# NSLab-CUK/LiteralKG

Measured on AMD Instinct MI355X. Metric: kg_edges_aggregated_per_sec, higher is better.
Workload: dtype f32

## Files before the change

include/literalkg_hip.h:

```cpp
#ifndef LITERALKG_HIP_H
#define LITERALKG_HIP_H

#include <stdint.h>

#ifdef __cplusplus
extern "C" {
#endif

typedef enum {
    LKG_OK = 0,
    LKG_ERR_INVALID_ARG = -1,
    LKG_ERR_HIP = -2,
    LKG_ERR_UNSUPPORTED = -3,
    LKG_ERR_NOMEM = -4
} lkg_status;

int lkg_version(void);
const char *lkg_last_error(void);
int lkg_preload(void);

int lkg_csr_build(int64_t n_entities, int64_t n_edges, const int64_t *h, const int64_t *t,
                  const int64_t *r, int32_t *rowptr, int32_t *col, int32_t *eptr, int32_t *rel,
                  int64_t *order, int64_t *nnz_out);

// ... 148 lines not shown

int lkg_gate_blend_fwd_f32(int64_t n, int32_t d, const float *x, int64_t ldx, const float *gpre,
                           int64_t ldg, const float *zpre, int64_t ldz, float *out, int64_t ldo,
                           void *stream);
int lkg_gate_blend_bwd_f32(int64_t n, int32_t d, const float *x, int64_t ldx, const float *gpre,
                           int64_t ldg, const float *zpre, int64_t ldz, const float *g_out,
                           int64_t ldgo, float *g_x, int64_t ldgx, float *g_gpre, int64_t ldgg,
                           float *g_zpre, int64_t ldgz, int32_t activated, float *g_pre_rowmax, void *stream);

int lkg_gate_blend_bwd_stats_f32(int64_t n, int32_t d, const float *x, int64_t ldx, const float *gpre, int64_t ldg,
                                 const float *zpre, int64_t ldz, const float *g_out, int64_t ldgo, float *g_x,
                                 int64_t ldgx, float *g_gpre, int64_t ldgg, float *g_zpre, int64_t ldgz,
                                 int32_t activated, float *g_pre_rowmax, const float *w, int64_t ldw, int32_t n_w,
                                 float *workspace, int64_t workspace_floats, float *stats, void *stream);

int lkg_gemm_wgrad_f32(int64_t m, int64_t n, int64_t k, const float *a, int64_t lda, const float *a_colmax,
                       const float *b, int64_t ldb, const float *b_colmax, float *c, int64_t ldc, void *stream);
int lkg_gemm_longk_ok(int64_t m, int64_t n, int64_t k, const float *a, int64_t lda, const float *b, int64_t ldb);
int lkg_gemm_longk_f32(int64_t m, int64_t n, int64_t k, const float *a, int64_t lda, const float *b, int64_t ldb,
                       float *c, int64_t ldc, void *stream);
int lkg_gemm_smallm_ok(int64_t m, int64_t n, int64_t k, const float *a, int64_t lda, const float *b, int64_t ldb);
int lkg_gemm_smallm_f32(int64_t m, int64_t n, int64_t k, const float *a, int64_t lda, const float *b, int64_t ldb,
                        float *c, int64_t ldc, void *stream);

int64_t lkg_narrow_layer_bwd_workspace(int64_t n);
int lkg_narrow_layer_bwd_ok(int64_t n, int32_t d_in, int32_t d_out, const float *x, int64_t ldx, const float *z, int64_t ldz,
                            const float *y, int64_t ldy, const float *g_y, int64_t ldgy, const float *g_yn, int64_t ldgyn);
int lkg_narrow_layer_bwd_f32(int64_t n, int32_t d_in, int32_t d_out, const float *x, int64_t ldx, const float *w, int64_t ldw,
                             const float *z, int64_t ldz, float slope, const float *gamma, const float *y, int64_t ldy,
                             const float *save_mean, const float *save_rstd, const float *g_y, int64_t ldgy,
                             const float *g_yn, int64_t ldgyn, float norm_eps, float drop_p, uint64_t seed,
                             const uint8_t *g_yn_rows, float *g_x, int64_t ldgx, float *g_w, float *g_bias,
                             float *g_gamma, float *g_beta, float *workspace, int64_t workspace_floats, void *stream);
int lkg_gemm_skinny_ok(int64_t m, int64_t n, int64_t k, const float *a, int64_t lda, const float *c, int64_t ldc);
int lkg_gemm_skinny_f32(int64_t m, int64_t n, int64_t k, const float *a, int64_t lda, const float *b, int64_t ldb,
                        int32_t trans_b, float beta, float *c, int64_t ldc, const float *bias, void *stream);
int lkg_col_absmax_f32(int64_t n, int32_t d, const float *x, int64_t ldx, float *out, void *stream);

int lkg_colsum_f32(int64_t n, int32_t d, const float *x, int64_t ldx, float *out, void *stream);
int lkg_colsum_weighted_f32(int64_t n, int32_t d, const float *x, int64_t ldx, const float *w, int64_t ldw,
                            int32_t n_w, float *out_sum, float *out_w, int64_t ld_out_w, void *stream);

int lkg_bi_mix_fwd_f32(int64_t n, int32_t d, const float *ego, int64_t lde, const float *side, int64_t lds,
                       const float *h0p, int64_t ldh, float alpha, float *out_sum, int64_t ldos, float *out_prod,
                       int64_t ldop, void *stream);
int lkg_bi_mix_bwd_f32(int64_t n, int32_t d, const float *ego, int64_t lde, const float *side, int64_t lds,
                       const float *g_sum, int64_t ldgs, const float *g_prod, int64_t ldgp, int32_t has_h0, float alpha,
                       float *g_ego, float *g_side, float *g_h0p, void *stream);

int lkg_eltwise_f32(int32_t op, int64_t n, int32_t d, const float *a, int64_t lda, const float *b,
                    int64_t ldb, float alpha, float beta, float *out, int64_t ldo, void *stream);

int lkg_adam_step_f32(int64_t n, float *param, const float *grad, float *exp_avg, float *exp_avg_sq,
                      float lr, float beta1, float beta2, float eps, float weight_decay, int64_t step,
                      void *stream);

int64_t lkg_gemm_workspace(int32_t trans_a, int64_t m, int64_t n, int64_t k);
int lkg_gemm_f32_engine(int32_t trans_a, int32_t trans_b, int64_t m, int64_t n, int64_t k, int64_t workspace_bytes);

int lkg_gemm_f64acc_f32(int32_t trans_a, int32_t trans_b, int64_t m, int64_t n, int64_t k, const float *a, int64_t lda,
                        const float *b, int64_t ldb, float *c, int64_t ldc, void *stream);
int lkg_gemm_f32(int32_t trans_a, int32_t trans_b, int64_t m, int64_t n, int64_t k, float alpha,
                 const float *a, int64_t lda, const float *b, int64_t ldb, float beta, float *c,
                 int64_t ldc, const float *bias, void *workspace, int64_t workspace_bytes, void *stream);

int lkg_row_absmax_f32(int64_t n, int32_t d, const float *x, int64_t ldx, float *out, int32_t accumulate,
// ... 78 lines not shown
```

literalkg_amd/_native.py:

```python
import ctypes as C
import os

_LIB_PATH = os.path.join(os.path.dirname(os.path.abspath(__file__)), "lib", "liblkg_hip.so")
_lib = None

i64, i32, f32, vp, u64 = C.c_int64, C.c_int32, C.c_float, C.c_void_p, C.c_uint64

PROTOTYPES = {
    "lkg_version": [],
    "lkg_last_error": [],
    "lkg_preload": [],
    "lkg_csr_build": [i64, i64, vp, vp, vp, vp, vp, vp, vp, vp, vp],
    "lkg_csr_transpose": [i64, i64, i64, vp, vp, vp, vp, vp],
    "lkg_row_partition": [i64, vp, i32, vp],
    "lkg_csr_coo_indices_i64": [i64, i64, vp, vp, vp, vp],
    "lkg_csr_build_device_workspace": [i64, i64],
    "lkg_csr_build_device": [i64, i64, vp, vp, vp, vp, vp, vp, vp, vp, vp, vp, i64, vp],
    "lkg_csr_transpose_device_workspace": [i64, i64],
    "lkg_csr_transpose_device": [i64, i64, i64, vp, vp, vp, vp, vp, vp, i64, vp],
    "lkg_triples_count": [C.c_char_p, vp],
    "lkg_triples_read": [C.c_char_p, i64, vp, vp, vp, vp],
    "lkg_triples_dedup": [i64, vp, vp, vp, vp, vp],
    "lkg_laplacian_f32": [i64, i64, i64, vp, vp, vp, vp, i32, vp],
    "lkg_laplacian_device_f32": [i64, i64, i32, vp, vp, vp, vp, i32, vp, vp, vp],
# ... 30 lines not shown
                                  vp, f32, u64, vp, vp, i32, vp, i64, vp],
    "lkg_dot_score_fwd_f32": [i64, i32, vp, i64, vp, vp, vp, vp, vp, vp, vp, vp],
    "lkg_dot_score_bwd_f32": [i64, i32, vp, i64, vp, vp, vp, vp, vp, f32, vp, vp, i64, vp],
    "lkg_relu_batchnorm_fwd_f32": [i64, i32, vp, i64, vp, vp, f32, i32, f32, vp, vp, vp, i64, vp, vp, vp],
    "lkg_relu_batchnorm_bwd_f32": [i64, i32, vp, i64, vp, vp, vp, i32, vp, i64, vp, i64, vp, vp, vp],
    "lkg_gate_blend_fwd_f32": [i64, i32, vp, i64, vp, i64, vp, i64, vp, i64, vp],
    "lkg_gate_blend_bwd_f32": [i64, i32, vp, i64, vp, i64, vp, i64, vp, i64, vp, i64, vp, i64, vp, i64, i32, vp, vp],
    "lkg_gate_blend_bwd_stats_f32": [i64, i32, vp, i64, vp, i64, vp, i64, vp, i64, vp, i64, vp, i64, vp, i64, i32, vp, vp,
                                     i64, i32, vp, i64, vp, vp],
    "lkg_row_absmax_f32": [i64, i32, vp, i64, vp, i32, vp],
    "lkg_gemm_tall_workspace": [i32, i32, vp, i32],
    "lkg_gemm_tall_f32": [i64, i32, i32, vp, vp, vp, vp, i32, vp, vp, i32, f32, f32, vp, i64, vp, i32, vp, i64, vp, i64,
                          vp, i64, vp, i64, vp],
    "lkg_linear_act_layernorm_workspace": [i32, i32, vp],
    "lkg_linear_act_layernorm_fwd_f32": [i64, i32, i32, vp, vp, vp, vp, vp, vp, vp, f32, vp, vp, f32, vp, i64, vp, i64, f32,
                                         vp, vp, f32, u64, vp, i64, vp],
    "lkg_gemm_workspace": [i32, i64, i64, i64],
    "lkg_gemm_f32_engine": [i32, i32, i64, i64, i64, i64],
    "lkg_gemm_f32": [i32, i32, i64, i64, i64, f32, vp, i64, vp, i64, f32, vp, i64, vp, vp, i64, vp],
    "lkg_gemm_f64acc_f32": [i32, i32, i64, i64, i64, vp, i64, vp, i64, vp, i64, vp],
    "lkg_colsum_f32": [i64, i32, vp, i64, vp, vp],
    "lkg_col_absmax_f32": [i64, i32, vp, i64, vp, vp],
    "lkg_gemm_longk_ok": [i64, i64, i64, vp, i64, vp, i64],
    "lkg_gemm_longk_f32": [i64, i64, i64, vp, i64, vp, i64, vp, i64, vp],
    "lkg_gemm_smallm_ok": [i64, i64, i64, vp, i64, vp, i64],
    "lkg_gemm_skinny_ok": [i64, i64, i64, vp, i64, vp, i64],
    "lkg_gemm_skinny_f32": [i64, i64, i64, vp, i64, vp, i64, i32, f32, vp, i64, vp, vp],
    "lkg_gemm_smallm_f32": [i64, i64, i64, vp, i64, vp, i64, vp, i64, vp],
    "lkg_gemm_wgrad_f32": [i64, i64, i64, vp, i64, vp, vp, i64, vp, vp, i64, vp],
    "lkg_narrow_layer_bwd_ok": [i64, i32, i32, vp, i64, vp, i64, vp, i64, vp, i64, vp, i64],
    "lkg_narrow_layer_bwd_workspace": [i64],
    "lkg_narrow_layer_bwd_f32": [i64, i32, i32, vp, i64, vp, i64, vp, i64, f32, vp, vp, i64, vp, vp, vp, i64, vp, i64, f32, f32,
                                 u64, vp, vp, i64, vp, vp, vp, vp, vp, i64, vp],
    "lkg_colsum_weighted_f32": [i64, i32, vp, i64, vp, i64, i32, vp, vp, i64, vp],
    "lkg_eltwise_f32": [i32, i64, i32, vp, i64, vp, i64, f32, f32, vp, i64, vp],
    "lkg_bi_mix_fwd_f32": [i64, i32, vp, i64, vp, i64, vp, i64, f32, vp, i64, vp, i64, vp],
    "lkg_bi_mix_bwd_f32": [i64, i32, vp, i64, vp, i64, vp, i64, vp, i64, i32, f32, vp, vp, vp, vp],
    "lkg_adam_step_f32": [i64, vp, vp, vp, vp, f32, f32, f32, f32, f32, i64, vp],
    "lkg_rank_sqnorm_f32": [i64, i32, vp, i64, vp, vp],
    "lkg_rank_queries_f32": [i64, i32, vp, i64, vp, vp, i64, vp, f32, vp, i64, vp],
    "lkg_rank_prepare_f32": [i64, i64, i32, vp, i64, vp, i64, vp, vp, vp, vp, vp, vp, vp, vp, vp, vp, vp, vp],
    "lkg_rank_count_f32": [i64, i64, i32, vp, i64, vp, i64, vp, vp, vp, vp, vp, vp],
    "lkg_topk_splits": [i64, i64, i32],
    "lkg_topk_select_f32": [i64, i64, i32, vp, i64, vp, i64, vp, vp, vp, vp, vp, vp, vp, vp, i32, i32, vp, vp, vp],
    "lkg_topk_merge_f32": [i64, i32, i32, vp, vp, vp, vp, vp, vp, vp],
    "lkg_pair_mlp_scores_f32": [i64, i64, vp, i64, vp, i64, vp, vp, vp, vp, vp, i64, vp],
    "lkg_pair_mlp_splits": [i64, i64, i32],
    "lkg_pair_mlp_select_f32": [i64, i64, vp, i64, vp, i64, vp, vp, vp, vp, vp, vp, vp, vp, vp, vp, vp, i32, i32, vp, vp,
                                vp],
    "lkg_pair_mlp_prepare_f32": [i64, i64, vp, i64, vp, i64, vp, vp, vp, vp, vp, i64, vp, vp, vp, vp, vp, vp, vp, vp, vp,
                                 vp, vp],
    "lkg_pair_mlp_count_f32": [i64, i64, vp, i64, vp, i64, vp, vp, vp, vp, vp, vp, vp, vp, vp],
    "lkg_pair_mlp_pairs_f32": [i64, vp, i64, vp, i64, vp, vp, vp, vp, vp, vp, vp, f32, vp, vp, vp],
    "lkg_binary_curve_workspace": [i64],
    "lkg_binary_curve_f32": [i64, vp, vp, vp, vp, vp, i64, vp],
    "lkg_triple_scores_f32": [i64, i32, vp, i64, vp, vp, vp, vp, i64, vp, f32, i32, vp, f32, vp, vp, vp],
    "lkg_threshold_fit_workspace": [i64, i64],
    "lkg_threshold_fit_f32": [i64, i64, vp, vp, vp, i32, vp, vp, vp, i64, vp],
}
_RESTYPE = {"lkg_last_error": C.c_char_p, "lkg_csr_build_device_workspace": C.c_int64,
            "lkg_gemm_tall_workspace": C.c_int64, "lkg_gemm_workspace": C.c_int64,
            "lkg_linear_act_layernorm_workspace": C.c_int64, "lkg_narrow_layer_bwd_workspace": C.c_int64,
            "lkg_csr_transpose_device_workspace": C.c_int64, "lkg_binary_curve_workspace": C.c_int64,
            "lkg_threshold_fit_workspace": C.c_int64}


# ... 70 lines not shown
```

literalkg_amd/csrc/lkg_spmm.hip:

```cpp
#include <stdlib.h>

#include <algorithm>
#include <type_traits>

#include "lkg_common.h"

namespace {

template <typename V>
struct vec_ops;
template <>
struct vec_ops<float4> {
    static constexpr int W = 4;
    static __device__ __forceinline__ float4 zero() { return f4_zero(); }
    static __device__ __forceinline__ void fma(float4 &a, float s, const float4 &x) { f4_fma(a, s, x); }
    static __device__ __forceinline__ float absmax(const float4 &a) {
        return fmaxf(fmaxf(fabsf(a.x), fabsf(a.y)), fmaxf(fabsf(a.z), fabsf(a.w)));
    }
    template <int M>
    static __device__ __forceinline__ void xor_add(float4 &a) {
        a.x = lane_xor_add<M>(a.x);
        a.y = lane_xor_add<M>(a.y);
        a.z = lane_xor_add<M>(a.z);
        a.w = lane_xor_add<M>(a.w);
// ... 229 lines not shown
            }
        }
        const V *csrc = ex.copy_dst ? reinterpret_cast<const V *>(ex.copy_src + (long)row * ex.ld_copy_src) : nullptr;
        V *cdst = ex.copy_dst ? reinterpret_cast<V *>(ex.copy_dst + (long)row * ex.ld_copy_dst) : nullptr;
#pragma unroll
        for (int i = 0; i < CPL; ++i) {
            const int chunk = lane + i * LPE;
            if (FULL || chunk < nchunk) {
                if (own) ops::fma(acc[i], 1.f, own[chunk]);
                if (own2) ops::fma(acc[i], 1.f, own2[chunk]);
#ifndef LKG_SPMM_PLAIN
                if constexpr (std::is_same<V, float4>::value) {
                    typedef float nt4 __attribute__((ext_vector_type(4)));
                    const nt4 nv = {acc[i].x, acc[i].y, acc[i].z, acc[i].w};
                    __builtin_nontemporal_store(nv, reinterpret_cast<nt4 *>(dst + chunk));
                } else {
                    __builtin_nontemporal_store(acc[i], dst + chunk);
                }
#else
                dst[chunk] = acc[i];
#endif
                if (cdst) cdst[chunk] = csrc[chunk];
                rmax = fmaxf(rmax, ops::absmax(acc[i]));
            }
        }
    }
    if (ex.rowmax) {
        rmax = wave_max(rmax);
        if (lane == 0) atomicMax(ex.rowmax + row, __float_as_int(rmax));
    }
}

template <typename V, int LPE, int U, bool FULL>
__global__ __launch_bounds__(256) void spmm_csr_grouped_kernel(int n_rows, int nchunk,
                                                                const int *__restrict__ rowptr,
                                                                const int *__restrict__ col,
                                                                const float *__restrict__ val,
                                                                const float *__restrict__ x, long ldx,
                                                                float *__restrict__ out, long ldo,
                                                                const float *__restrict__ self, long ld_self,
                                                                const int *__restrict__ long_rows, int n_long,
                                                                int long_thresh, SpmmExtra ex) {
    using ops = vec_ops<V>;
    static_assert(LPE <= 32 && LPE % U == 0, "grouped SpMM: 2+ rows per wave, whole U-groups per chunk");
    __shared__ V part[4][LPE];
    const int lane = threadIdx.x & 63, w = threadIdx.x >> 6;
    if ((int)blockIdx.x < n_long) {
        const int row = long_rows[blockIdx.x];
        const int start = __builtin_amdgcn_readfirstlane(rowptr[row]);
        const int end = __builtin_amdgcn_readfirstlane(rowptr[row + 1]);
        V acc[1] = {ops::zero()};
        accumulate_entries<V, LPE, 1, U, FULL>(acc, start, end, w, 4, lane, nchunk, col, val, x, ldx);
        reduce_subgroups<V, LPE>(acc[0]);
        if (lane < LPE) part[w][lane] = acc[0];
        __syncthreads();
        if (w != 0 || lane >= LPE || !(FULL || lane < nchunk)) return;
        V a = part[0][lane];
#pragma unroll
        for (int k = 1; k < 4; ++k) ops::fma(a, 1.f, part[k][lane]);
        if (self) ops::fma(a, 1.f, reinterpret_cast<const V *>(self + (long)row * ld_self)[lane]);
        if (const float *a2 = ex.add2_row(row)) ops::fma(a, 1.f, reinterpret_cast<const V *>(a2)[lane]);
        reinterpret_cast<V *>(out + (long)row * ldo)[lane] = a;
        if (ex.rowmax) atomicMax(ex.rowmax + row, __float_as_int(ops::absmax(a)));
        if (ex.copy_dst)
            reinterpret_cast<V *>(ex.copy_dst + (long)row * ex.ld_copy_dst)[lane] =
                reinterpret_cast<const V *>(ex.copy_src + (long)row * ex.ld_copy_src)[lane];
        return;
    }
    constexpr int RPW = 64 / LPE;
    const int sub = lane / LPE, sl = lane % LPE;
    const int slot = (((int)blockIdx.x - n_long) * 4 + w) * RPW + sub;
    const bool valid = slot < n_rows;
    const int row = valid ? slot : 0;
    int start = 0, len = 0;
    if (valid) {
        start = rowptr[row];
        len = rowptr[row + 1] - start;
    }
    const bool mine = valid && !(n_long > 0 && len > long_thresh);
    if (!mine) len = 0;
    int maxlen = len;
    int spare = len > 0 ? start : -1;
#pragma unroll
    for (int m = LPE; m < 64; m <<= 1) {
        maxlen = max(maxlen, __shfl_xor(maxlen, m, 64));
        spare = max(spare, __shfl_xor(spare, m, 64));
    }
    V acc = ops::zero();
    for (int k = 0; k < maxlen; k += LPE) {
        const int j = k + sl;
        const int jc = len > 0 ? start + min(j, len - 1) : spare;
        const int c = col[jc];
        const float v = j < len ? val[jc] : 0.f;
        const int mcnt = min(LPE, maxlen - k);
        for (int q = 0; q < mcnt; q += U) {
            int cc[U];
            float vv[U];
            V xv[U];
#pragma unroll
            for (int u = 0; u < U; ++u) {
                cc[u] = __shfl(c, sub * LPE + q + u, 64);
                vv[u] = __shfl(v, sub * LPE + q + u, 64);
            }
#pragma unroll
            for (int u = 0; u < U; ++u) {
                const V *src = reinterpret_cast<const V *>(x + (long)cc[u] * ldx);
                xv[u] = FULL ? src[sl] : src[min(sl, nchunk - 1)];
            }
#pragma unroll
            for (int u = 0; u < U; ++u) ops::fma(acc, vv[u], xv[u]);
        }
    }
    const bool writes = mine && (FULL || sl < nchunk);
    if (writes) {
        if (len == 0) acc = ops::zero();
        if (self) ops::fma(acc, 1.f, reinterpret_cast<const V *>(self + (long)row * ld_self)[sl]);
        if (const float *a2 = ex.add2_row(row)) ops::fma(acc, 1.f, reinterpret_cast<const V *>(a2)[sl]);
        reinterpret_cast<V *>(out + (long)row * ldo)[sl] = acc;
        if (ex.copy_dst)
            reinterpret_cast<V *>(ex.copy_dst + (long)row * ex.ld_copy_dst)[sl] =
                reinterpret_cast<const V *>(ex.copy_src + (long)row * ex.ld_copy_src)[sl];
    }
    if (ex.rowmax) {
        const float rm = group_max<LPE>(writes ? ops::absmax(acc) : 0.f);
        if (mine && sl == 0) atomicMax(ex.rowmax + row, __float_as_int(rm));
    }
}

template <int CPL, bool FULL>
__global__ __launch_bounds__(256) void spmm_flagged4_kernel(int n_rows, int nchunk, const int *__restrict__ rowptr,
                                                             const int *__restrict__ col, const float *__restrict__ val,
                                                             const float *__restrict__ x, long ldx,
                                                             float *__restrict__ out, long ldo,
                                                             const float *__restrict__ self, long ld_self, int n_long,
                                                             int long_thresh, SpmmExtra ex) {
    const int lane = threadIdx.x & 63, q = lane >> 4, ql = lane & 15;
    const int task = (int)blockIdx.x * 4 + (threadIdx.x >> 6);
    const int row_q = task * 4 + q;
    int start = 0, len = 0;
    if (row_q < n_rows) {
        start = rowptr[row_q];
        len = rowptr[row_q + 1] - start;
        if (n_long > 0 && len > long_thresh) len = 0;
    }
    int maxlen = len;
    maxlen = max(maxlen, __shfl_xor(maxlen, 16, 64));
    maxlen = max(maxlen, __shfl_xor(maxlen, 32, 64));
    float4 acc[4][CPL];
#pragma unroll
    for (int r = 0; r < 4; ++r)
#pragma unroll
        for (int i = 0; i < CPL; ++i) acc[r][i] = f4_zero();
    unsigned any = 0;
    for (int p = 0; p < maxlen; p += 16) {
        const int j = p + ql;
        const bool in = j < len;
        const int jj = start + (in ? j : 0);
        const int c = len > 0 ? col[jj] : 0;
        unsigned long long m = __ballot(in && ex.x_rows[c] != 0);
// ... 258 lines not shown
        return LKG_OK;
    }
    const int block_cols = (vec && !x_rows) ? 128 : 256;
    const bool grouped_slabs = vec && !x_rows && block_cols / 4 <= LKG_SPMM_GROUPED_CHUNKS;
    if (d > block_cols && d % block_cols == 0 && !grouped_slabs)
        return vec ? dispatch<float4>(n_rows, block_cols / 4, rowptr, col, val, x, ldx, out, ldo, self, ld_self,
                                      long_rows, n_long, long_thresh, d / block_cols, block_cols, ex, s)
                   : dispatch<float>(n_rows, block_cols, rowptr, col, val, x, ldx, out, ldo, self, ld_self, long_rows,
                                     n_long, long_thresh, d / block_cols, block_cols, ex, s);
    for (int c0 = 0; c0 < d; c0 += block_cols) {
        const int dc = min(block_cols, d - c0);
        const SpmmExtra exc{add2 ? add2 + c0 : nullptr, (long)ld_add2, add2 ? add2_rows : nullptr,
                            copy_dst ? copy_src + c0 : nullptr,
                            (long)ld_copy_src, copy_dst ? copy_dst + c0 : nullptr, (long)ld_copy_dst,
                            reinterpret_cast<int *>(rowmax_out), x_rows, self ? self_rows : nullptr, out_rows, ex.row_list, ex.n_list};
        int rc = vec ? dispatch<float4>(n_rows, dc / 4, rowptr, col, val, x + c0, ldx, out + c0, ldo,
                                        self ? self + c0 : nullptr, ld_self, long_rows, n_long, long_thresh, 1, 0, exc, s)
                     : dispatch<float>(n_rows, dc, rowptr, col, val, x + c0, ldx, out + c0, ldo,
                                       self ? self + c0 : nullptr, ld_self, long_rows, n_long, long_thresh, 1, 0, exc, s);
        if (rc != LKG_OK) return rc;
    }
    return LKG_OK;
}

extern "C" int lkg_spmm_csr_f32(int64_t n_rows, int32_t d, const int32_t *rowptr, const int32_t *col,
                                const float *val, const float *x, int64_t ldx, float *out, int64_t ldo,
                                const float *self, int64_t ld_self, const int32_t *long_rows, int32_t n_long,
                                int32_t long_thresh, void *stream) {
    return lkg_spmm_csr_fused_f32(n_rows, d, rowptr, col, val, x, ldx, out, ldo, self, ld_self, nullptr, 0, nullptr,
                                  nullptr, 0, nullptr, 0, nullptr, nullptr, nullptr, nullptr, long_rows, n_long, long_thresh,
                                  nullptr, 0, nullptr, 0, stream);
}

__global__ void permute_kernel(long n, long n_src, const int *__restrict__ perm, const float *__restrict__ src,
                               float *__restrict__ dst) {
    long i = (long)blockIdx.x * blockDim.x + threadIdx.x;
    const long stride = (long)gridDim.x * blockDim.x;
    for (; i < n; i += stride) {
        const long p = perm[i];
        dst[i] = (p >= 0 && p < n_src) ? src[p] : __builtin_nanf("");
    }
}

extern "C" int lkg_permute_f32(int64_t n, const int32_t *perm, int64_t n_src, const float *src, float *dst, void *stream) {
    LKG_REQUIRE(n >= 0 && n_src >= 0, "lkg_permute_f32: negative extent");
    if (n == 0) return LKG_OK;
    LKG_REQUIRE(perm && src && dst, "lkg_permute_f32: null pointer");
    const int64_t blocks = std::min<int64_t>((n + 255) / 256, 256 * 8);
    hipLaunchKernelGGL(permute_kernel, dim3((unsigned)blocks), dim3(256), 0, (hipStream_t)stream, (long)n, (long)n_src, perm,
                       src, dst);
    LKG_CHECK_LAUNCH("lkg_permute_f32");
    return LKG_OK;
}

__global__ __launch_bounds__(256) void csr_check_kernel(long n_rows, const int *__restrict__ rowptr, long nnz,
                                                        const int *__restrict__ col, long col_offset, long n_cols,
                                                        int *__restrict__ bad) {
    const long stride = (long)gridDim.x * blockDim.x;
    const long t0 = (long)blockIdx.x * blockDim.x + threadIdx.x;
    int mine = 0;
    for (long i = t0; i < n_rows; i += stride) {
        const long a = rowptr[i], b = rowptr[i + 1];
        mine += (a < 0 || a > b || b > nnz) ? 1 : 0;
    }
    long lo = rowptr[0], hi = rowptr[n_rows];
    lo = lo < 0 ? 0 : (lo > nnz ? nnz : lo);
// ... 89 lines not shown
```

literalkg_amd/model.py:

```python
from __future__ import annotations

import math
import os
from typing import Optional

import torch
import torch.nn as nn

from . import ops, pruned
from .gate import Gate, GateMul
from .graph import KGStructure


class AttentionCSR:

    def __init__(self, graph: KGStructure, val: torch.Tensor, val_t: Optional[torch.Tensor] = None):
        self.graph = graph
        self.val = val
        self.val_t = val_t if val_t is not None else (
            ops.permute_values(val, graph.t_perm) if graph.t_perm is not None and val.is_cuda else None)

    def aggregate(self, ego: torch.Tensor, plus_self: bool = False, bias: Optional[torch.Tensor] = None) -> torch.Tensor:
        return ops.aggregate(ego, self.graph, self.val, self.val_t, plus_self, bias)

# ... 103 lines not shown
                                  want_y=self.want_output)
        self.last_normalized = yn
        return y

    def _linear_finish(self, xs, ws, bias):
        ln = self.layer_normalize
        if len(xs) == 1 and ops.narrow_layer_ok(xs[0], ws[0]):
            p = float(self.dropout) if self.training else 0.0
            y, yn = ops.narrow_layer(xs[0], ws[0], bias, ln.weight, ln.bias, want_norm=True, drop_p=p, yn_out=self.norm_out,
                                     want_y=self.want_output)
            self.last_normalized = yn
            return y
        if ops.fused_layer_wanted(xs, ws, (bias, ln.weight, ln.bias)):
            p = float(self.dropout) if self.training else 0.0
            y, yn = ops.linear_act_layernorm(xs, ws, bias, ln.weight, ln.bias, want_norm=True, drop_p=p, yn_out=self.norm_out,
                                             want_y=self.want_output)
            self.last_normalized = yn
            return y
        return self._finish(ops.multi_linear(xs, ws, bias))

    def narrows(self) -> bool:
        return self.aggregator_type == "gcn" and not self.use_residual and 2 * self.out_dim <= self.in_dim

    def forward(self, ego_embeddings, A_in: AttentionCSR, all_layers, lamda, alpha, l):
        ego = ego_embeddings
        h0 = all_layers[0]
        kind = self.aggregator_type
        if kind == "gcn":
            att = getattr(A_in, "att", A_in)
            if self.narrows() and isinstance(att, AttentionCSR):
                p = ops.linear(ego, self.linear.weight, None)
                return self._finish(att.aggregate(p, True, bias=self.linear.bias))
            if not self.use_residual:
                return self._linear_finish((A_in.aggregate(ego, True),), (self.linear.weight,), self.linear.bias)
            z = self._res_lin(self.linear, A_in.aggregate(ego, True), h0, lamda, alpha, l)
            return self._finish(z)
        if kind == "gin":
            return self._gin(ego, A_in.aggregate(ego, True), h0, all_layers, lamda, alpha, l)
        side = A_in.aggregate(ego)
        if kind == "graphsage":
            if self.use_residual:
                wh = self.linear_h.weight
                hi = ops.multi_linear((ego, side), (wh[:, :self.in_dim], wh[:, self.in_dim:]), self.linear_h.bias)
                z = self._res_lin(self.linear, hi, h0, lamda, alpha, l)
            else:
                w = self.linear.weight
                return self._linear_finish((ego, side), (w[:, :self.in_dim], w[:, self.in_dim:]), self.linear.bias)
            return self._finish(z)
        if kind == "bi-interaction":
            h0p = None
            if self.use_residual:
                h0p = self.h0_projection if self.h0_projection is not None else \
                    ops.linear(h0, self.linear_h0.weight, self.linear_h0.bias)
            ms, mp = ops.bi_mix(ego, side, h0p, alpha)
            if self.use_residual:
                wp = self._identity_map(lamda, l)
                s, b = self._lin_mapped(self.linear1, ms, wp), self._lin_mapped(self.linear2, mp, wp)
            else:
                s, b = self._lin(self.linear1, ms), self._lin(self.linear2, mp)
            return self._finish(ops.leaky_relu_sum(b, s), slope=1.0)
        raise NotImplementedError(kind)

    def _gin(self, ego, ego_plus_side, h0, all_layers, lamda, alpha, l):
        if self.num_layers == 1:
            raise AttributeError("gin with n_mlp_layers == 1 cannot run in the reference either "
                                 "(inp_linear/out_linear are never created, model.py:66-68, 133)")
# ... 470 lines not shown
```

literalkg_amd/ops.py:

```python
from __future__ import annotations

from typing import Optional, Sequence, Tuple

import torch
from torch.autograd import Function

from . import _native as N
from .graph import KGStructure, LONG_ROW_THRESHOLD

LEAKY_SLOPE = 0.01
LN_EPS = 1e-5
NORMALIZE_EPS = 1e-12


_raw_stream = getattr(torch._C, "_cuda_getCurrentRawStream", None)


def _stream():
    if _raw_stream is not None:
        return _raw_stream(torch.cuda.current_device())
    return torch.cuda.current_stream().cuda_stream


def _need_gpu(*ts):
# ... 1256 lines not shown
            ids = rows.compact_ids()
            zc = None
            for x, w in zip(xs, ws):
                zc = gemm(gather_rows_range(x, ids, 0, n), w, trans_b=True, beta=0.0 if zc is None else 1.0, out=zc,
                          bias=bias if zc is None else None)
            keep = ids >= 0
            z = torch.empty((n, d), dtype=torch.float32, device=zc.device)
            z.index_copy_(0, ids[keep], zc[keep])
        elif tall_ok(n, d, [x.shape[1] for x in xs], single_panel_too=True):
            z = gemm_tall(xs, (ws,), True, bias)
        else:
            z = None
            for x, w in zip(xs, ws):
                z = gemm(x, w, trans_b=True, beta=0.0 if z is None else 1.0, out=z, bias=bias if z is None else None)
        gz, gg, gb = _ActLayerNorm.backward(_ShimCtx((z, gamma, beta, mean, rstd, *([y] if y is not None else [])), cfg=cfg),
                                            gy, gyn)[:3]
        need = ctx.needs_input_grad
        lin = _MultiLinear.backward(_ShimCtx((*xs, *ws), n_terms=n_terms, has_bias=has_bias,
                                             needs_input_grad=(need[0], False, *need[12:12 + 2 * n_terms])), gz)
        return (lin[0], gg, gb) + none[3:] + tuple(lin[2:])


def linear_act_layernorm(xs: Sequence[torch.Tensor], ws: Sequence[torch.Tensor], bias, gamma, beta, want_norm=True,
                         slope=LEAKY_SLOPE, eps=LN_EPS, norm_eps=NORMALIZE_EPS, drop_p: float = 0.0,
                         seed: Optional[int] = None, yn_out: Optional[torch.Tensor] = None, want_y: bool = True):
    if drop_p > 0 and seed is None:
        seed = new_seed()
    return _FusedLayer.apply(bias, gamma, beta, len(xs), float(slope), float(eps), float(norm_eps), float(drop_p), seed or 0,
                             yn_out, want_y, want_norm, *xs, *ws)


NARROW_LAYER = _os.environ.get("LKG_NARROW_LAYER", "1") not in ("", "0")
"""Run the DENSE backward of a 32 -> 32 aggregation layer's Linear + LeakyReLU + LayerNorm (+ dropout + normalised copy) as one
launch (lkg_narrow_layer_bwd_f32) instead of four (row-wise backward, data gradient, weight gradient, bias column sum).  The
forward launches, and the backward under row-sparse gradients, are the unfused pair's own."""


def narrow_layer_ok(x: torch.Tensor, w: torch.Tensor) -> bool:
    return (NARROW_LAYER and x.is_cuda and x.dim() == 2 and x.shape[1] == 32 and tuple(w.shape) == (32, 32) and x.shape[0] >= 4096
            and _skinny(x, 32))


class _NarrowLayer(Function):

    @staticmethod
    def forward(ctx, x, w, bias, gamma, beta, want_norm, slope, eps, norm_eps, drop_p, seed, yn_out, want_y):
        _need_gpu(x, w, gamma, beta)
        x = _f32_rows(x)
        z = gemm(x, w, trans_b=True, bias=bias)
        n, d = z.shape
        if not want_y and not want_norm:
            raise ValueError("narrow_layer: neither output wanted")
        y = torch.empty((n, d), dtype=torch.float32, device=z.device) if want_y else None
        yn = None
        if want_norm:
            yn = yn_out if yn_out is not None else torch.empty((n, d), dtype=torch.float32, device=z.device)
        mean = torch.empty(n, dtype=torch.float32, device=z.device)
        rstd = torch.empty(n, dtype=torch.float32, device=z.device)
        N.call("lkg_act_layernorm_fwd_f32", n, d, N.ptr(z), _ld(z), float(slope), N.ptr(gamma), N.ptr(beta),
               float(eps), N.ptr(y), _ld(y) if y is not None else 0, N.ptr(yn), _ld(yn) if yn is not None else 0,
               float(norm_eps), N.ptr(mean), N.ptr(rstd), float(drop_p), int(seed), _stream())
        ctx.save_for_backward(x, w, z, gamma, beta, mean, rstd, *([y] if y is not None else []))
        ctx.cfg = (slope, norm_eps, drop_p, seed)
        ctx.has_bias = bias is not None
        ctx.set_materialize_grads(False)
        return y, yn

    @staticmethod
# ... 9 lines not shown
        rows_n, rows_y = tagged_rows(gyn), tagged_rows(gy)
        rows = union_rows(rows_y, rows_n) if (gy is None or rows_y is not None) and (gyn is None or rows_n is not None) else None
        gy_ = _f32_rows(gy) if gy is not None else None
        gyn_ = _f32_rows(gyn) if gyn is not None else None
        fused = (not rows_worth_compacting(rows, n) and need[0] and need[1] and gamma.data_ptr() % 16 == 0
                 and N.load().lkg_narrow_layer_bwd_ok(n, x.shape[1], d, N.ptr(x), _ld(x), N.ptr(z), _ld(z), N.ptr(y),
                                                      _ld(y) if y is not None else 0, N.ptr(gy_), _ld(gy_) if gy_ is not None else 0,
                                                      N.ptr(gyn_), _ld(gyn_) if gyn_ is not None else 0))
        if not fused:
            gz, gg, gb = _ActLayerNorm.backward(_ShimCtx((z, gamma, beta, mean, rstd, *kept_y), cfg=ctx.cfg), gy, gyn)[:3]
            lin = _MultiLinear.backward(_ShimCtx((x, w), n_terms=1, has_bias=ctx.has_bias,
                                                 needs_input_grad=(need[2], False, need[0], need[1])), gz)
            return (lin[2], lin[3], lin[0], gg, gb) + none[5:]
        gx = torch.empty((n, x.shape[1]), dtype=torch.float32, device=z.device)
        sums = torch.empty(32 * 32 + 3 * 32, dtype=torch.float32, device=z.device)
        gw, gbias, gg, gb = sums[:1024].view(32, 32), sums[1024:1056], sums[1056:1088], sums[1088:1120]
        wc = w if w.stride(1) == 1 else w.contiguous()
        ws_floats = int(N.load().lkg_narrow_layer_bwd_workspace(n))
        ws_ = _workspace(4 * ws_floats, z.device)
        N.call("lkg_narrow_layer_bwd_f32", n, x.shape[1], d, N.ptr(x), _ld(x), N.ptr(wc), _ld(wc), N.ptr(z), _ld(z), float(slope),
               N.ptr(gamma), N.ptr(y), _ld(y) if y is not None else 0, N.ptr(mean), N.ptr(rstd), N.ptr(gy_),
               _ld(gy_) if gy_ is not None else 0, N.ptr(gyn_), _ld(gyn_) if gyn_ is not None else 0, float(norm_eps), float(drop_p),
               int(seed), N.ptr(_flags(rows_n)) if gyn_ is not None else None, N.ptr(gx), _ld(gx), N.ptr(gw),
               N.ptr(gbias) if (ctx.has_bias and need[2]) else None, N.ptr(gg), N.ptr(gb), N.ptr(ws_), ws_floats, _stream())
        return (gx, gw, gbias if (ctx.has_bias and need[2]) else None, gg, gb) + none[5:]


def narrow_layer(x, w, bias, gamma, beta, want_norm=True, slope=LEAKY_SLOPE, eps=LN_EPS, norm_eps=NORMALIZE_EPS,
                 drop_p: float = 0.0, seed: Optional[int] = None, yn_out: Optional[torch.Tensor] = None, want_y: bool = True):
    if drop_p > 0 and seed is None:
        seed = new_seed()
    return _NarrowLayer.apply(x, w, bias, gamma, beta, want_norm, float(slope), float(eps), float(norm_eps), float(drop_p),
                              seed or 0, yn_out, want_y)


class CatBuffer:

    def __init__(self, n: int, widths: Sequence[int], device):
        self.widths = list(widths)
        self.offsets = [0]
        for w in self.widths:
            self.offsets.append(self.offsets[-1] + w)
        self.buf = torch.empty((n, self.offsets[-1]), dtype=torch.float32, device=device)

    def slot(self, k: int) -> torch.Tensor:
        return self.buf[:, self.offsets[k]:self.offsets[k + 1]]


def _same_view(a: torch.Tensor, b: torch.Tensor) -> bool:
    return (a.data_ptr() == b.data_ptr() and a.shape == b.shape
            and all(sa == sb for sa, sb, n_ in zip(a.stride(), b.stride(), a.shape) if n_ > 1))


class _AssembleCat(Function):
    @staticmethod
    def forward(ctx, holder: CatBuffer, pending, *parts):
        for k, p in enumerate(parts):
            s = holder.slot(k)
            if k in pending:
                continue
            if not _same_view(p, s):
                s.copy_(p)
        ctx.offsets = holder.offsets
        return holder.buf.detach()

    @staticmethod
# ... 878 lines not shown
```

Baseline: 6.653 billion.

## Fuse CSR aggregation, 32x32 linear and layer-norm into one forward kernel

```diff
diff --git a/include/literalkg_hip.h b/include/literalkg_hip.h
--- a/include/literalkg_hip.h
+++ b/include/literalkg_hip.h
@@ -204,6 +204,16 @@
                              const float *g_yn, int64_t ldgyn, float norm_eps, float drop_p, uint64_t seed,
                              const uint8_t *g_yn_rows, float *g_x, int64_t ldgx, float *g_w, float *g_bias,
                              float *g_gamma, float *g_beta, float *workspace, int64_t workspace_floats, void *stream);
+int lkg_agg_narrow_layer_fwd_ok(int64_t n_rows, int32_t d_in, int32_t d_out, const float *src, int64_t ld_src,
+                                const float *ego, int64_t ld_ego, const float *x, int64_t ldx, const float *z, int64_t ldz,
+                                const float *y, int64_t ldy, const float *yn, int64_t ldyn);
+int lkg_agg_narrow_layer_fwd_f32(int64_t n_rows, int32_t d_in, int32_t d_out, const int32_t *rowptr, const int32_t *col,
+                                 const float *val, const float *src, int64_t ld_src, const float *ego, int64_t ld_ego,
+                                 const int32_t *long_rows, int32_t n_long, int32_t long_thresh, const float *w, int64_t ldw,
+                                 const float *bias, float slope, const float *gamma, const float *beta, float eps, float *x,
+                                 int64_t ldx, float *z, int64_t ldz, float *y, int64_t ldy, float *yn, int64_t ldyn,
+                                 float norm_eps, float *save_mean, float *save_rstd, float drop_p, uint64_t seed,
+                                 void *stream);
 int lkg_gemm_skinny_ok(int64_t m, int64_t n, int64_t k, const float *a, int64_t lda, const float *c, int64_t ldc);
 int lkg_gemm_skinny_f32(int64_t m, int64_t n, int64_t k, const float *a, int64_t lda, const float *b, int64_t ldb,
                         int32_t trans_b, float beta, float *c, int64_t ldc, const float *bias, void *stream);
diff --git a/literalkg_amd/_native.py b/literalkg_amd/_native.py
--- a/literalkg_amd/_native.py
+++ b/literalkg_amd/_native.py
@@ -86,6 +86,9 @@
     "lkg_narrow_layer_bwd_workspace": [i64],
     "lkg_narrow_layer_bwd_f32": [i64, i32, i32, vp, i64, vp, i64, vp, i64, f32, vp, vp, i64, vp, vp, vp, i64, vp, i64, f32, f32,
                                  u64, vp, vp, i64, vp, vp, vp, vp, vp, i64, vp],
+    "lkg_agg_narrow_layer_fwd_ok": [i64, i32, i32, vp, i64, vp, i64, vp, i64, vp, i64, vp, i64, vp, i64],
+    "lkg_agg_narrow_layer_fwd_f32": [i64, i32, i32, vp, vp, vp, vp, i64, vp, i64, vp, i32, i32, vp, i64, vp, f32, vp, vp, f32,
+                                     vp, i64, vp, i64, vp, i64, vp, i64, f32, vp, vp, f32, u64, vp],
     "lkg_colsum_weighted_f32": [i64, i32, vp, i64, vp, i64, i32, vp, vp, i64, vp],
     "lkg_eltwise_f32": [i32, i64, i32, vp, i64, vp, i64, f32, f32, vp, i64, vp],
     "lkg_bi_mix_fwd_f32": [i64, i32, vp, i64, vp, i64, vp, i64, f32, vp, i64, vp, i64, vp],
diff --git a/literalkg_amd/csrc/lkg_spmm.hip b/literalkg_amd/csrc/lkg_spmm.hip
--- a/literalkg_amd/csrc/lkg_spmm.hip
+++ b/literalkg_amd/csrc/lkg_spmm.hip
@@ -285,6 +285,46 @@
 }
 
 template <typename V, int LPE, int U, bool FULL>
+__device__ __forceinline__ V accumulate_grouped_rows(int start, int len, int lane, int nchunk, const int *__restrict__ col,
+                                                     const float *__restrict__ val, const float *__restrict__ x, long ldx) {
+    using ops = vec_ops<V>;
+    const int sub = lane / LPE, sl = lane % LPE;
+    int maxlen = len;
+    int spare = len > 0 ? start : -1;
+#pragma unroll
+    for (int m = LPE; m < 64; m <<= 1) {
+        maxlen = max(maxlen, __shfl_xor(maxlen, m, 64));
+        spare = max(spare, __shfl_xor(spare, m, 64));
+    }
+    V acc = ops::zero();
+    for (int k = 0; k < maxlen; k += LPE) {
+        const int j = k + sl;
+        const int jc = len > 0 ? start + min(j, len - 1) : spare;
+        const int c = col[jc];
+        const float v = j < len ? val[jc] : 0.f;
+        const int mcnt = min(LPE, maxlen - k);
+        for (int q = 0; q < mcnt; q += U) {
+            int cc[U];
+            float vv[U];
+            V xv[U];
+#pragma unroll
+            for (int u = 0; u < U; ++u) {
+                cc[u] = __shfl(c, sub * LPE + q + u, 64);
+                vv[u] = __shfl(v, sub * LPE + q + u, 64);
+            }
+#pragma unroll
+            for (int u = 0; u < U; ++u) {
+                const V *src = reinterpret_cast<const V *>(x + (long)cc[u] * ldx);
+                xv[u] = FULL ? src[sl] : src[min(sl, nchunk - 1)];
+            }
+#pragma unroll
+            for (int u = 0; u < U; ++u) ops::fma(acc, vv[u], xv[u]);
+        }
+    }
+    return acc;
+}
+
+template <typename V, int LPE, int U, bool FULL>
 __global__ __launch_bounds__(256) void spmm_csr_grouped_kernel(int n_rows, int nchunk,
                                                                 const int *__restrict__ rowptr,
                                                                 const int *__restrict__ col,
@@ -332,38 +372,7 @@
     }
     const bool mine = valid && !(n_long > 0 && len > long_thresh);
     if (!mine) len = 0;
-    int maxlen = len;
-    int spare = len > 0 ? start : -1;
-#pragma unroll
-    for (int m = LPE; m < 64; m <<= 1) {
-        maxlen = max(maxlen, __shfl_xor(maxlen, m, 64));
-        spare = max(spare, __shfl_xor(spare, m, 64));
-    }
-    V acc = ops::zero();
-    for (int k = 0; k < maxlen; k += LPE) {
-        const int j = k + sl;
-        const int jc = len > 0 ? start + min(j, len - 1) : spare;
-        const int c = col[jc];
-        const float v = j < len ? val[jc] : 0.f;
-        const int mcnt = min(LPE, maxlen - k);
-        for (int q = 0; q < mcnt; q += U) {
-            int cc[U];
-            float vv[U];
-            V xv[U];
-#pragma unroll
-            for (int u = 0; u < U; ++u) {
-                cc[u] = __shfl(c, sub * LPE + q + u, 64);
-                vv[u] = __shfl(v, sub * LPE + q + u, 64);
-            }
-#pragma unroll
-            for (int u = 0; u < U; ++u) {
-                const V *src = reinterpret_cast<const V *>(x + (long)cc[u] * ldx);
-                xv[u] = FULL ? src[sl] : src[min(sl, nchunk - 1)];
-            }
-#pragma unroll
-            for (int u = 0; u < U; ++u) ops::fma(acc, vv[u], xv[u]);
-        }
-    }
+    V acc = accumulate_grouped_rows<V, LPE, U, FULL>(start, len, lane, nchunk, col, val, x, ldx);
     const bool writes = mine && (FULL || sl < nchunk);
     if (writes) {
         if (len == 0) acc = ops::zero();
@@ -378,6 +387,146 @@
         const float rm = group_max<LPE>(writes ? ops::absmax(acc) : 0.f);
         if (mine && sl == 0) atomicMax(ex.rowmax + row, __float_as_int(rm));
     }
+}
+
+struct NarrowLayerOut {
+    const float *w;
+    long ldw;
+    const float *bias;
+    const float *gamma, *beta;
+    float slope, eps, norm_eps, drop_p;
+    unsigned long long seed;
+    float *x, *z, *y, *yn;
+    long ldx, ldz, ldy, ldyn;
+    float *mean, *rstd;
+    int d;
+};
+
+__device__ __forceinline__ void narrow_layer_row(const float4 &xa, long row, bool stores, int lane, const float (*ws)[32],
+                                                 const float *bias_s, const NarrowLayerOut &o) {
+    const int sl = lane & 7, base = lane & ~7;
+    const int e = sl * 4;
+    const int d = o.d;
+    const bool live = e < d;
+    if (o.x && stores) *reinterpret_cast<float4 *>(o.x + row * o.ldx + e) = xa;
+    const float xe[4] = {xa.x, xa.y, xa.z, xa.w};
+    float a[4];
+    {
+        const float4 bv = *reinterpret_cast<const float4 *>(bias_s + e);
+        a[0] = bv.x; a[1] = bv.y; a[2] = bv.z; a[3] = bv.w;
+    }
+#pragma unroll
+    for (int q = 0; q < 8; ++q)
+#pragma unroll
+        for (int k = 0; k < 4; ++k) {
+            const float xk = __shfl(xe[k], base + q, 64);
+            const float4 wv = *reinterpret_cast<const float4 *>(&ws[4 * q + k][e]);
+            a[0] = fmaf(xk, wv.x, a[0]);
+            a[1] = fmaf(xk, wv.y, a[1]);
+            a[2] = fmaf(xk, wv.z, a[2]);
+            a[3] = fmaf(xk, wv.w, a[3]);
+        }
+    if (o.z && stores) *reinterpret_cast<float4 *>(o.z + row * o.ldz + e) = make_float4(a[0], a[1], a[2], a[3]);
+    float g[4], b[4];
+    {
+        const float4 gg = *reinterpret_cast<const float4 *>(o.gamma + e);
+        const float4 bb = *reinterpret_cast<const float4 *>(o.beta + e);
+        g[0] = gg.x; g[1] = gg.y; g[2] = gg.z; g[3] = gg.w;
+        b[0] = bb.x; b[1] = bb.y; b[2] = bb.z; b[3] = bb.w;
+    }
+    float s = 0.f;
+#pragma unroll
+    for (int k = 0; k < 4; ++k) {
+        const float t = a[k];
+        a[k] = t > 0.f ? t : t * o.slope;
+        s += live ? a[k] : 0.f;
+    }
+    const float mean = group_sum<8>(s) / (float)d;
+    float q = 0.f;
+#pragma unroll
+    for (int k = 0; k < 4; ++k) {
+        const float c = live ? a[k] - mean : 0.f;
+        q = fmaf(c, c, q);
+    }
+    const float rstd = 1.f / sqrtf(group_sum<8>(q) / (float)d + o.eps);
+    float nn = 0.f;
+    const float drop_p = o.drop_p;
+    const float inv_keep = drop_p > 0.f ? 1.f / (1.f - drop_p) : 1.f;
+    const unsigned rkey = drop_row_key(o.seed, (unsigned long long)row);
+#pragma unroll
+    for (int k = 0; k < 4; ++k) {
+        float v = (a[k] - mean) * rstd * g[k] + b[k];
+        if (drop_p > 0.f) v *= drop_scale(rkey, (unsigned)(e + k), drop_p, inv_keep);
+        a[k] = v;
+        nn += live ? v * v : 0.f;
+    }
+    if (o.y && stores && live) *reinterpret_cast<float4 *>(o.y + row * o.ldy + e) = make_float4(a[0], a[1], a[2], a[3]);
+    if (sl == 0 && stores) {
+        o.mean[row] = mean;
+        o.rstd[row] = rstd;
+    }
+    if (o.yn) {
+        const float inv = 1.f / fmaxf(sqrtf(group_sum<8>(nn)), o.norm_eps);
+        if (stores && live)
+            *reinterpret_cast<float4 *>(o.yn + row * o.ldyn + e) = make_float4(a[0] * inv, a[1] * inv, a[2] * inv, a[3] * inv);
+    }
+}
+
+__global__ __launch_bounds__(256) void agg_narrow_layer_fwd_kernel(int n_rows, const int *__restrict__ rowptr,
+                                                                    const int *__restrict__ col,
+                                                                    const float *__restrict__ val,
+                                                                    const float *__restrict__ src, long ld_src,
+                                                                    const float *__restrict__ ego, long ld_ego,
+                                                                    const int *__restrict__ long_rows, int n_long,
+                                                                    int long_thresh, NarrowLayerOut o) {
+    constexpr int LPE = 8, U = 8, RPW = 64 / LPE;
+    __shared__ __attribute__((aligned(16))) float ws[32][32], bias_s[32];
+    __shared__ float4 part[4][LPE];
+    const int lane = threadIdx.x & 63, w = threadIdx.x >> 6;
+    const int sl = lane % LPE;
+    const bool team = (int)blockIdx.x < n_long;
+    const float4 wreg = *reinterpret_cast<const float4 *>(o.w + (long)(threadIdx.x >> 3) * o.ldw + 4 * (threadIdx.x & 7));
+    const float breg = (threadIdx.x < 32 && o.bias) ? o.bias[threadIdx.x] : 0.f;
+    const int slot = team ? 0 : (((int)blockIdx.x - n_long) * 4 + w) * RPW + lane / LPE;
+    const bool valid = !team && slot < n_rows;
+    const int row = valid ? slot : 0;
+    int start = 0, len = 0;
+    if (valid) {
+        start = rowptr[row];
+        len = rowptr[row + 1] - start;
+    }
+    {
+        const int wc = threadIdx.x >> 3, wk = 4 * (threadIdx.x & 7);
+        ws[wk][wc] = wreg.x;
+        ws[wk + 1][wc] = wreg.y;
+        ws[wk + 2][wc] = wreg.z;
+        ws[wk + 3][wc] = wreg.w;
+        if (threadIdx.x < 32) bias_s[threadIdx.x] = breg;
+    }
+    __syncthreads();
+    if (team) {
+        const int lrow = long_rows[blockIdx.x];
+        const int lstart = __builtin_amdgcn_readfirstlane(rowptr[lrow]);
+        const int lend = __builtin_amdgcn_readfirstlane(rowptr[lrow + 1]);
+        float4 acc[1] = {f4_zero()};
+        accumulate_entries<float4, LPE, 1, U, true>(acc, lstart, lend, w, 4, lane, LPE, col, val, src, ld_src);
+        reduce_subgroups<float4, LPE>(acc[0]);
+        if (lane < LPE) part[w][lane] = acc[0];
+        __syncthreads();
+        if (w != 0) return;
+        float4 a = part[0][sl];
+#pragma unroll
+        for (int k = 1; k < 4; ++k) f4_fma(a, 1.f, part[k][sl]);
+        f4_fma(a, 1.f, reinterpret_cast<const float4 *>(ego + (long)lrow * ld_ego)[sl]);
+        narrow_layer_row(a, lrow, lane < LPE, lane, ws, bias_s, o);
+        return;
+    }
+    const bool mine = valid && !(n_long > 0 && len > long_thresh);
+    if (!mine) len = 0;
+    float4 acc = accumulate_grouped_rows<float4, LPE, U, true>(start, len, lane, LPE, col, val, src, ld_src);
+    if (len == 0) acc = f4_zero();
+    f4_fma(acc, 1.f, reinterpret_cast<const float4 *>(ego + (long)row * ld_ego)[sl]);
+    narrow_layer_row(acc, row, mine, lane, ws, bias_s, o);
 }
 
 template <int CPL, bool FULL>
@@ -702,6 +851,41 @@
                                   nullptr, 0, nullptr, 0, stream);
 }
 
+extern "C" int lkg_agg_narrow_layer_fwd_ok(int64_t n_rows, int32_t d_in, int32_t d_out, const float *src, int64_t ld_src,
+                                           const float *ego, int64_t ld_ego, const float *x, int64_t ldx, const float *z,
+                                           int64_t ldz, const float *y, int64_t ldy, const float *yn, int64_t ldyn) {
+    return n_rows > 0 && n_rows < INT32_MAX - 64 && d_in == 32 && d_out == 32 && src && ego && ld_src >= 32 && ld_ego >= 32 &&
+           ld_src % 4 == 0 && ld_ego % 4 == 0 && lkg_aligned16(src) && lkg_aligned16(ego) &&
+           (!x || (ldx >= 32 && ldx % 4 == 0 && lkg_aligned16(x))) && (!z || (ldz >= 32 && ldz % 4 == 0 && lkg_aligned16(z))) &&
+           (!y || (ldy >= 32 && ldy % 4 == 0 && lkg_aligned16(y))) && (!yn || (ldyn >= 32 && ldyn % 4 == 0 && lkg_aligned16(yn)));
+}
+
+extern "C" int lkg_agg_narrow_layer_fwd_f32(int64_t n_rows, int32_t d_in, int32_t d_out, const int32_t *rowptr, const int32_t *col,
+                                            const float *val, const float *src, int64_t ld_src, const float *ego, int64_t ld_ego,
+                                            const int32_t *long_rows, int32_t n_long, int32_t long_thresh, const float *w,
+                                            int64_t ldw, const float *bias, float slope, const float *gamma, const float *beta,
+                                            float eps, float *x, int64_t ldx, float *z, int64_t ldz, float *y, int64_t ldy,
+                                            float *yn, int64_t ldyn, float norm_eps, float *save_mean, float *save_rstd,
+                                            float drop_p, uint64_t seed, void *stream) {
+    LKG_REQUIRE(rowptr && col && val && src && ego && w && gamma && beta && save_mean && save_rstd,
+                "lkg_agg_narrow_layer_fwd_f32: null pointer");
+    LKG_REQUIRE(lkg_agg_narrow_layer_fwd_ok(n_rows, d_in, d_out, src, ld_src, ego, ld_ego, x, ldx, z, ldz, y, ldy, yn, ldyn) &&
+                ldw >= 32 && ldw % 4 == 0 && lkg_aligned16(w) && lkg_aligned16(gamma) && lkg_aligned16(beta),
+                "lkg_agg_narrow_layer_fwd_f32: needs 32 columns in and out, at least one row and 16-byte aligned rows of at least "
+                "32 floats (lkg_agg_narrow_layer_fwd_ok)");
+    LKG_REQUIRE(drop_p >= 0.f && drop_p < 1.f, "lkg_agg_narrow_layer_fwd_f32: drop_p outside [0, 1)");
+    LKG_REQUIRE(n_long >= 0 && (n_long == 0 || (long_rows && long_thresh >= 64)),
+                "lkg_agg_narrow_layer_fwd_f32: long-row list needs a pointer and a threshold >= 64");
+    const int64_t blocks = (n_rows + 31) / 32 + n_long;
+    LKG_REQUIRE(blocks * 256 < (int64_t)UINT32_MAX, "lkg_agg_narrow_layer_fwd_f32: grid too large (%lld workgroups)", (long long)blocks);
+    const NarrowLayerOut o{w, (long)ldw, bias, gamma, beta, slope, eps, norm_eps, drop_p, (unsigned long long)seed, x, z, y, yn,
+                           (long)ldx, (long)ldz, (long)ldy, (long)ldyn, save_mean, save_rstd, 32};
+    hipLaunchKernelGGL(agg_narrow_layer_fwd_kernel, dim3((unsigned)blocks), dim3(256), 0, (hipStream_t)stream, (int)n_rows, rowptr,
+                       col, val, src, (long)ld_src, ego, (long)ld_ego, long_rows, n_long, long_thresh, o);
+    LKG_CHECK_LAUNCH("lkg_agg_narrow_layer_fwd_f32");
+    return LKG_OK;
+}
+
 __global__ void permute_kernel(long n, long n_src, const int *__restrict__ perm, const float *__restrict__ src,
                                float *__restrict__ dst) {
     long i = (long)blockIdx.x * blockDim.x + threadIdx.x;
diff --git a/literalkg_amd/model.py b/literalkg_amd/model.py
--- a/literalkg_amd/model.py
+++ b/literalkg_amd/model.py
@@ -159,6 +159,14 @@
                 p = ops.linear(ego, self.linear.weight, None)
                 return self._finish(att.aggregate(p, True, bias=self.linear.bias))
             if not self.use_residual:
+                if type(A_in) is AttentionCSR and ops.agg_narrow_layer_ok(ego, A_in.graph, self.linear.weight):
+                    ln = self.layer_normalize
+                    p = float(self.dropout) if self.training else 0.0
+                    y, yn = ops.agg_narrow_layer(ego, A_in.graph, A_in.val, A_in.val_t, self.linear.weight, self.linear.bias,
+                                                 ln.weight, ln.bias, want_norm=True, drop_p=p, yn_out=self.norm_out,
+                                                 want_y=self.want_output)
+                    self.last_normalized = yn
+                    return y
                 return self._linear_finish((A_in.aggregate(ego, True),), (self.linear.weight,), self.linear.bias)
             z = self._res_lin(self.linear, A_in.aggregate(ego, True), h0, lamda, alpha, l)
             return self._finish(z)
diff --git a/literalkg_amd/ops.py b/literalkg_amd/ops.py
--- a/literalkg_amd/ops.py
+++ b/literalkg_amd/ops.py
@@ -1312,8 +1312,11 @@
 
 NARROW_LAYER = _os.environ.get("LKG_NARROW_LAYER", "1") not in ("", "0")
 """Run the DENSE backward of a 32 -> 32 aggregation layer's Linear + LeakyReLU + LayerNorm (+ dropout + normalised copy) as one
-launch (lkg_narrow_layer_bwd_f32) instead of four (row-wise backward, data gradient, weight gradient, bias column sum).  The
-forward launches, and the backward under row-sparse gradients, are the unfused pair's own."""
+launch (lkg_narrow_layer_bwd_f32) instead of four (row-wise backward, data gradient, weight gradient, bias column sum), and the
+FORWARD of such a gcn layer over a plain CSR -- aggregation, Linear and the row-wise kernel -- as one launch instead of three
+(lkg_agg_narrow_layer_fwd_f32, agg_narrow_layer: same bits; x and z are stored only when a backward will read them).  The
+backward under row-sparse gradients is the unfused pair's own; every other layer shape keeps its launches.  LKG_NARROW_LAYER=0
+selects the unfused launches throughout (A/B runs)."""
 
 
 def narrow_layer_ok(x: torch.Tensor, w: torch.Tensor) -> bool:
@@ -1389,6 +1392,71 @@
         seed = new_seed()
     return _NarrowLayer.apply(x, w, bias, gamma, beta, want_norm, float(slope), float(eps), float(norm_eps), float(drop_p),
                               seed or 0, yn_out, want_y)
+
+
+def agg_narrow_layer_ok(ego: torch.Tensor, g, w: torch.Tensor) -> bool:
+    return (narrow_layer_ok(ego, w) and isinstance(g, KGStructure) and g.rowptr is not None and g.rowptr.is_cuda
+            and ego.shape[0] == g.n and tagged_rows(ego) is None and g.row_lists(False) is None)
+
+
+class _AggNarrowLayer(Function):
+
+    @staticmethod
+    def forward(ctx, ego, g: KGStructure, val, val_t, w, bias, gamma, beta, want_norm, slope, eps, norm_eps, drop_p, seed,
+                yn_out, want_y, keep):
+        _need_gpu(ego, val, w, gamma, beta, bias)
+        _check_table(ego, g, val)
+        if not want_y and not want_norm:
+            raise ValueError("agg_narrow_layer: neither output wanted")
+        ego = _f32_rows(ego)
+        n, d = g.n, w.shape[0]
+        if CHECK_STRUCTURES:
+            check_csr(g.rowptr, g.col, n, n, what="agg_narrow_layer")
+        dev = ego.device
+        new = lambda *shape: torch.empty(shape, dtype=torch.float32, device=dev)
+        x, z = (new(n, d), new(n, d)) if keep else (None, None)
+        y = new(n, d) if want_y else None
+        yn = (yn_out if yn_out is not None else new(n, d)) if want_norm else None
+        mean, rstd = new(n), new(n)
+        wc = w.detach() if w.stride(1) == 1 else w.detach().contiguous()
+        bc = bias.detach().contiguous() if bias is not None else None
+        long_rows = g.long_rows(False)
+        ld = lambda t: _ld(t) if t is not None else 0
+        N.call("lkg_agg_narrow_layer_fwd_f32", n, ego.shape[1], d, N.ptr(g.rowptr), N.ptr(g.col), N.ptr(val), N.ptr(ego), _ld(ego),
+               N.ptr(ego), _ld(ego), N.ptr(long_rows), 0 if long_rows is None else long_rows.numel(), LONG_ROW_THRESHOLD,
+               N.ptr(wc), _ld(wc), N.ptr(bc), float(slope), N.ptr(gamma), N.ptr(beta), float(eps), N.ptr(x), ld(x), N.ptr(z), ld(z),
+               N.ptr(y), ld(y), N.ptr(yn), ld(yn), float(norm_eps), N.ptr(mean), N.ptr(rstd), float(drop_p), int(seed), _stream())
+        if keep:
+            ctx.save_for_backward(x, w, z, gamma, beta, mean, rstd, *([y] if y is not None else []))
+        ctx.g, ctx.val_t = g, val_t
+        ctx.cfg = (slope, norm_eps, drop_p, seed)
+        ctx.has_bias = bias is not None
+        ctx.set_materialize_grads(False)
+        return y, yn
+
+    @staticmethod
+    def backward(ctx, gy, gyn):
+        none = (None,) * 17
+        if gy is None and gyn is None:
+            return none
+        need = ctx.needs_input_grad
+        dense = _NarrowLayer.backward(_ShimCtx(ctx.saved_tensors, cfg=ctx.cfg, has_bias=ctx.has_bias,
+                                               needs_input_grad=(need[0], need[4], need[5])), gy, gyn)
+        gx, gw, gbias, gg, gb = dense[:5]
+        g_ego = None
+        if need[0] and gx is not None:
+            g_ego = _Aggregate._backward_ego(_ShimCtx((), g=ctx.g, val_t=ctx.val_t, plus_self=True), gx)[0]
+        return (g_ego, None, None, None, gw, gbias, gg, gb) + none[8:]
+
+
+def agg_narrow_layer(ego, g: KGStructure, val, val_t, w, bias, gamma, beta, want_norm=True, slope=LEAKY_SLOPE, eps=LN_EPS,
+                     norm_eps=NORMALIZE_EPS, drop_p: float = 0.0, seed: Optional[int] = None,
+                     yn_out: Optional[torch.Tensor] = None, want_y: bool = True):
+    if drop_p > 0 and seed is None:
+        seed = new_seed()
+    keep = torch.is_grad_enabled() and any(t is not None and t.requires_grad for t in (ego, w, bias, gamma, beta))
+    return _AggNarrowLayer.apply(ego, g, val, val_t, w, bias, gamma, beta, want_norm, float(slope), float(eps), float(norm_eps),
+                                 float(drop_p), seed or 0, yn_out, want_y, keep)
 
 
 class CatBuffer:
```

Result: no change. 6.648 billion (-0.1%).
